# yoozzeek/zk-lisp

Hardware: AMD Instinct MI355X
Metric: segment-proofs/sec at 65536 rows, blowup=16; proof bytes bit-exact vs CPU ref (higher is better)
Workload: dtype f128 (u128 mod 2^128-45*2^40+1)

## Files before the change

### include/zkl_hip.h

```cpp
#ifndef ZKL_HIP_H
#define ZKL_HIP_H

#include <stddef.h>
#include <stdint.h>

#ifdef __cplusplus
extern "C" {
#endif

#define ZKL_ABI_VERSION 1

enum {
  ZKL_OK = 0,
  ZKL_E_INVALID = -1,
  ZKL_E_DEVICE = -2,
  ZKL_E_OOM = -3,
  ZKL_E_INTERNAL = -4,
};

typedef struct { uint64_t lo, hi; } zkl_f128;

typedef struct {
  uint32_t num_queries;
  uint32_t blowup_factor;
// ... 118 lines not shown
int zkl_hip_kernel_times(const zkl_ctx* ctx, double* out_ms, int* out_launches, int max_n, const char** names);
int zkl_hip_set_kernel_timing(zkl_ctx* ctx, int mode);

int zkl_hip_device_count(int* count);
int zkl_hip_device_alloc(zkl_ctx* ctx, size_t bytes, void** d_ptr);
int zkl_hip_device_free(zkl_ctx* ctx, void* d_ptr);
int zkl_hip_memcpy(zkl_ctx* ctx, void* dst, const void* src, size_t bytes, int kind);
int zkl_hip_synchronize(zkl_ctx* ctx);

void zkl_select_partitions(uint32_t trace_width, uint32_t trace_length,
                           uint32_t* num_partitions, uint32_t* hash_rate);

int zkl_hip_hash_rows(zkl_ctx* ctx, const void* d_matrix, uint32_t n_cols, uint32_t n_rows,
                      uint32_t num_partitions, uint32_t hash_rate, void* d_digests_out);
int zkl_hip_merkle_tree(zkl_ctx* ctx, const void* d_leaves, uint32_t n_leaves, void* d_nodes_out);
int zkl_hip_poseidon_permute(zkl_ctx* ctx, void* d_states, uint32_t n_states, int engine);
int zkl_hip_set_hash_policy(int engine, uint32_t pm_min_items);
int zkl_hip_set_row_digest_rule(int rule);
int zkl_hip_row_digest_rule(void);
int zkl_hip_set_ntt_mode(int mode);
int zkl_hip_lde(zkl_ctx* ctx, const void* d_values, uint32_t n_cols, uint32_t n_rows,
                uint32_t blowup, void* d_coeffs_out, void* d_lde_out);

#define ZKL_COL_GENERAL 0xFFFFFFFFu
int zkl_hip_set_column_structure(int on);
int zkl_hip_column_structure(void);
int zkl_hip_scan_columns(zkl_ctx* ctx, const void* d_matrix, uint32_t n_cols, uint32_t n_rows, uint32_t* period_out);
int zkl_hip_plan_row_prefix(const uint32_t* period, uint32_t n_cols, uint64_t n_lde_rows, uint32_t blowup,
                            uint32_t num_partitions, uint32_t hash_rate, uint32_t* lead_out, uint32_t* q_out,
                            uint32_t* n_parts_out);
int zkl_hip_plan_row_zero_mask(const uint32_t* period, uint32_t n_cols, uint32_t num_partitions, uint32_t hash_rate,
                               uint64_t* even_out, uint64_t* odd_out, uint32_t* n_parts_out);
int zkl_hip_set_row_zero_mask(int on);
int zkl_hip_row_zero_mask(void);
int zkl_hip_hash_rows_periodic(zkl_ctx* ctx, const void* d_matrix, uint32_t n_cols, uint32_t n_rows,
                               uint32_t num_partitions, uint32_t hash_rate, const uint32_t* row_period, int split,
                               void* d_digests_out, uint32_t* resumed_out);
int zkl_hip_lde_columns(zkl_ctx* ctx, const void* d_values, uint32_t n_cols, uint32_t n_rows, uint32_t blowup,
                        const uint32_t* period, int want_split, void* d_coeffs_out, void* d_lde_out, int* split_out);

int zkl_hip_ntt(zkl_ctx* ctx, void* d_data, uint32_t n_cols, uint32_t n, int dif, int inverse);

int zkl_verify_segment(const uint8_t* proof, size_t len, const zkl_air_public_inputs* pi,
                       const zkl_proof_options* opts);

int zkl_synth_vm_segment(uint64_t seed, uint32_t log_n, zkl_f128* trace_out,
                         zkl_air_public_inputs* pi_out, uint32_t* width_out);
#define ZKL_SYN_SPONGE 1u
#define ZKL_SYN_RAM 2u
#define ZKL_SYN_MERKLE 4u
int zkl_synth_vm_segment_ex(uint64_t seed, uint32_t log_n, uint32_t flags, zkl_f128* trace_out,
                            zkl_air_public_inputs* pi_out, uint32_t* width_out);
int zkl_synth_vm_segment_chain(uint64_t program_seed, uint64_t seed, uint32_t log_n, uint32_t flags, const zkl_f128* rom0_in,
                               zkl_f128* trace_out, zkl_air_public_inputs* pi_out, uint32_t* width_out);

enum {
  ZKL_OP_CONST = 0, ZKL_OP_MOV, ZKL_OP_ADD, ZKL_OP_SUB, ZKL_OP_MUL, ZKL_OP_NEG, ZKL_OP_EQ, ZKL_OP_SELECT,
  ZKL_OP_ASSERT, ZKL_OP_ASSERT_BIT, ZKL_OP_ASSERT_RANGE, ZKL_OP_ASSERT_RANGE_LO, ZKL_OP_ASSERT_RANGE_HI,
  ZKL_OP_DIVMOD, ZKL_OP_DIVMOD128, ZKL_OP_MULWIDE, ZKL_OP_LOAD, ZKL_OP_STORE, ZKL_OP_SABSORBN, ZKL_OP_SSQUEEZE,
  ZKL_OP_MERKLE_FIRST, ZKL_OP_MERKLE_STEP, ZKL_OP_MERKLE_LAST, ZKL_OP_END
// ... 78 lines not shown
```

### zk-lisp_amd/csrc/kernels.h

```cpp
#pragma once
#include <hip/hip_runtime.h>
#include <stdint.h>

#include <stdexcept>
#include <string>
#include "air_host.h"
#include "field.h"

namespace zkl {

struct DeviceError : std::runtime_error { using std::runtime_error::runtime_error; };
#define ZKL_HIPCHECK(x)                                                                       \
  do {                                                                                        \
    hipError_t e_ = (x);                                                                      \
    if (e_ != hipSuccess) throw ::zkl::DeviceError(std::string(#x) + ": " + hipGetErrorString(e_)); \
  } while (0)
inline void check_launch(const char* what) {
  const hipError_t e = hipGetLastError();
  if (e != hipSuccess) throw DeviceError(std::string("kernel launch failed (") + what + "): " + hipGetErrorString(e));
}

struct HasherConsts {
  fe mds[144];
  fe rc[27 * 12];
// ... 44 lines not shown
                         bool clear = true);
void decode_column_scan(const uint32_t* bits, uint32_t n_cols, size_t n_rows, uint32_t* period);
struct RowPrefixPlan {
  uint32_t np = 0;
  uint32_t lead[16] = {0};
  uint32_t q[16] = {0};
  uint64_t zeven[16] = {0};
  uint64_t zodd[16] = {0};
  bool any() const {
    for (uint32_t p = 0; p < np; p++)
      if (lead[p]) return true;
    return false;
  }
};
constexpr uint32_t ROW_MASK_PAIRS = 64;
bool row_zero_mask_enabled();
void set_row_zero_mask(bool on);
RowPrefixPlan plan_row_prefix(const uint32_t* period, uint32_t n_cols, size_t n_rows, uint32_t blowup,
                              uint32_t num_partitions, uint32_t hash_rate, size_t rows_per_entry = 64);
size_t row_prefix_table_bytes(const RowPrefixPlan& plan);
bool launch_hash_rows_prefix(const fe* d_mat, uint32_t n_cols, size_t n_rows, uint32_t num_partitions,
                             uint32_t hash_rate, const RowPrefixPlan& plan, uint32_t* d_table, fe* d_tmp, fe* d_out,
                             hipStream_t s, int split = 0);
struct OpenRowJob { uint32_t src, dst; };
struct MergeNodeJob { uint32_t left, right, dst; };
void launch_open_rows(fe* d_buf, const OpenRowJob* d_jobs, size_t njobs, uint32_t ncols, uint32_t psize, uint32_t merge,
                      hipStream_t s);
void launch_merge_jobs(fe* d_buf, const MergeNodeJob* d_jobs, size_t njobs, hipStream_t s);
void launch_merkle(fe* d_nodes, size_t n_leaves, hipStream_t s, fe* d_coin = nullptr, fe* d_root_out = nullptr,
                   int coin_mode = 0);
void launch_draws(fe seed, uint64_t base, size_t k, fe* d_out, hipStream_t s, const fe* d_seed = nullptr);
void launch_grind(fe seed, uint64_t base, uint32_t count, uint32_t bits, unsigned long long* d_best, hipStream_t s,
                  const fe* d_seed = nullptr);
void launch_fri_remainder(const fe* d_ev, uint32_t Nr, uint32_t rlen, const fe* wk, const fe* sk, fe* d_coin,
                          fe* d_rem, hipStream_t s);
void launch_query_seed(fe* d_coin, const unsigned long long* d_best, hipStream_t s);

struct MontTab {
  const uint4* l4;
  const uint32_t* l1;
};
void build_mont_table(const fe* h_w, size_t N, void* d_buf, hipStream_t s);
inline MontTab mont_tab(const void* d_buf, size_t N) {
  return MontTab{(const uint4*)d_buf, (const uint32_t*)((const char*)d_buf + N * 16)};
}
void launch_ntt_stages(fe* d_data, size_t n_cols, size_t N, bool dif, int lo_log, int hi_log,
// ... 42 lines not shown
  CeParams ce;
  fe alpha[1024];
};
struct DerivedConsts {
  fe pose_k[27];
  fe apre[1025];
  fe deep[512];
  uint32_t deep_m[512][5];
  fe deep_sz[2];
};
void launch_constraint_eval(const fe* d_lde, const fe* d_roots, size_t Ntab, const fe* d_pertab,
                            const fe* d_bm , const CeParams& p, ProofConsts* dK,
                            const DerivedConsts* dD, bool pose_block, bool ram_merkle,
                            fe* d_xinv , bool xinv_ready, fe* d_out,
                            hipStream_t s, int split = 0, fe* d_pose_part  = nullptr);
void launch_check_rows(const fe* d_trace, size_t n, const fe* d_rowper, const ProofConsts* dK, const DerivedConsts* dD,
                       bool pose_block, bool ram_merkle, fe* d_pose_part, uint32_t* d_min, hipStream_t s);
void launch_check_assertions(const fe* d_trace, size_t n, const uint32_t* d_col, const uint32_t* d_step,
                             const fe* d_val, size_t n_assert, uint32_t* d_min, hipStream_t s);
void launch_boundary_scatter(const uint32_t* d_slot, const uint32_t* d_step, const fe* d_beta, size_t n_assert,
                             size_t n, fe* d_vecs, hipStream_t s);
void launch_boundary_w(const uint32_t* d_row_start, const fe* d_beta, const fe* d_val, size_t n, fe* d_w, hipStream_t s);
void launch_check_zero_range_bitrev(const fe* d_data, size_t N, size_t lo, size_t hi, unsigned* d_flag, hipStream_t s);

struct OodArgs {
  const fe* coef;
  size_t col_stride, elem_stride, n;
  const fe* pw1;
  const fe* pw2;
  uint32_t ncols, chunks, use_off;
  uint32_t off[16];
  const uint32_t* zero;
};
void launch_ood(const OodArgs& a, fe* d_partial, hipStream_t s);
void launch_ood_frame(const fe* d_partial_trace, const fe* d_partial_comp, uint32_t W, uint32_t C, uint32_t chunks,
                      const fe* mult , fe* d_frame, hipStream_t s);
struct DeepParams {
  size_t N;
  uint32_t W, C;
  fe z, zg;
};
void launch_deep_denoms(const fe* d_roots, size_t Ntab, size_t N, fe z, fe zg, fe* d_dinv, hipStream_t s);
void launch_deep(const fe* d_lde, const fe* d_clde, const fe* d_roots, size_t Ntab, const DeepParams& p,
                 const DerivedConsts* dD, const fe* d_dinv , fe* d_out, hipStream_t s,
                 int split = 0, const uint32_t* d_list = nullptr, uint32_t n_list = 0);
void launch_fri_leaves(const fe* d_ev, size_t Nd, fe* d_leaves, hipStream_t s);
// ... 6 lines not shown
```

### zk-lisp_amd/csrc/kernels.hip

```cpp
#include <hip/hip_runtime.h>

#include <algorithm>
#include <atomic>
#include <cstdlib>
#include <cstring>
#include <map>
#include <mutex>
#include <set>
#include <stdexcept>
#include <vector>

#include "kernels.h"
#include "air_eval.h"
#include "mont26.h"

namespace zkl {


void upload_air_consts(ProofConsts* dK, const AirDevice& a, hipStream_t s) {
  ZKL_HIPCHECK(hipMemcpyAsync(&dK->air, &a, sizeof a, hipMemcpyHostToDevice, s));
}
void upload_alphas_from_device(ProofConsts* dK, const fe* d, int n, hipStream_t s) {
  if (n > 1024) throw std::invalid_argument("more than 1024 transition constraints");
  ZKL_HIPCHECK(hipMemcpyAsync(dK->alpha, d, sizeof(fe) * n, hipMemcpyDeviceToDevice, s));
// ... 1142 lines not shown
  boundary_scatter_kernel<<<(unsigned)((na + 255) / 256), 256, 0, s>>>(d_slot, d_step, d_beta, na, n, d_vecs);
}
__global__ void boundary_w_kernel(const uint32_t* rs, const fe* beta, const fe* val, size_t n, fe* w) {
  size_t row = (size_t)blockIdx.x * blockDim.x + threadIdx.x;
  if (row >= n) return;
  uint32_t acc[9] = {0, 0, 0, 0, 0, 0, 0, 0, 0};
  for (uint32_t a = rs[row]; a < rs[row + 1]; a++) mul_acc(beta[a], val[a], acc);
  w[row] = reduce288(acc);
}
void launch_boundary_w(const uint32_t* d_rs, const fe* d_beta, const fe* d_val, size_t n, fe* d_w, hipStream_t s) {
  boundary_w_kernel<<<(unsigned)((n + 255) / 256), 256, 0, s>>>(d_rs, d_beta, d_val, n, d_w);
}

__global__ void check_zero_kernel(const fe* d, size_t N, int logN, size_t lo, size_t hi, unsigned* flag) {
  size_t k = lo + (size_t)blockIdx.x * blockDim.x + threadIdx.x;
  if (k >= hi) return;
  fe v = d[bitrev((uint32_t)k, logN)];
  if (!fe_is_zero(v)) atomicOr(flag, 1u);
}
void launch_check_zero_range_bitrev(const fe* d, size_t N, size_t lo, size_t hi, unsigned* flag, hipStream_t s) {
  if (hi > lo) check_zero_kernel<<<(unsigned)((hi - lo + 255) / 256), 256, 0, s>>>(d, N, ilog2s(N), lo, hi, flag);
}

__global__ __launch_bounds__(256) void ood_kernel(OodArgs A, fe* partial) {
  const uint32_t c = blockIdx.x, k = blockIdx.z;
  if (A.zero && A.zero[c]) {
    if (threadIdx.x < 2) partial[((size_t)threadIdx.x * A.ncols + c) * A.chunks + k] = fe_zero();
    return;
  }
  const fe* col = A.coef + (A.use_off ? (size_t)A.off[c] : (size_t)c * A.col_stride);
  const size_t len = A.n / A.chunks, j0 = (size_t)k * len;
  uint32_t acc1[9] = {0, 0, 0, 0, 0, 0, 0, 0, 0}, acc2[9] = {0, 0, 0, 0, 0, 0, 0, 0, 0};
  for (size_t j = j0 + threadIdx.x; j < j0 + len; j += 256) {
    const fe v = col[j * A.elem_stride];
    mul_acc(v, A.pw1[j], acc1);
    mul_acc(v, A.pw2[j], acc2);
  }
  __shared__ fe red[2][256];
  red[0][threadIdx.x] = reduce288(acc1);
  red[1][threadIdx.x] = reduce288(acc2);
  __syncthreads();
  for (int w = 128; w > 0; w >>= 1) {
    if ((int)threadIdx.x < w) {
      red[0][threadIdx.x] = fe_add(red[0][threadIdx.x], red[0][threadIdx.x + w]);
      red[1][threadIdx.x] = fe_add(red[1][threadIdx.x], red[1][threadIdx.x + w]);
    }
// ... 187 lines not shown
```

### zk-lisp_amd/csrc/poseidon.hip

```cpp
#include <hip/hip_runtime.h>

#include <algorithm>
#include <atomic>
#include <cstdio>
#include <cstdlib>
#include <cstring>
#include <mutex>
#include <stdexcept>
#include <vector>

#include "kernels.h"
#include "mont26.h"

namespace zkl {

__constant__ HasherMont c_hm;

__device__ __forceinline__ void to_mont130(fe a, uint32_t out[5]) {
  uint32_t l[5];
  to26(a, l);
  uint64_t col[10] = {0, 0, 0, 0, 0, 0, 0, 0, 0, 0};
  mac5(l, c_hm.r2_130, col);
  redc130(col, out);
}
// ... 534 lines not shown
          if (P == COL_GENERAL || (P & (P - 1))) { ok = false; break; }
          bp = std::max<uint64_t>(bp, P);
        }
      if (!ok) break;
      lead++;
      pmax = std::max(pmax, bp);
    }
    const uint64_t q = pmax > 1 ? pmax * blowup : 1;
    if (lead && q <= nrows / rows_per_entry && (q & (q - 1)) == 0) {
      pl.lead[p] = lead;
      pl.q[p] = (uint32_t)q;
    }
  }
  return pl;
}

size_t row_prefix_table_bytes(const RowPrefixPlan& pl) {
  size_t e = 0;
  for (uint32_t p = 0; p < pl.np; p++)
    if (pl.lead[p]) e += pl.q[p];
  return e * PM_PFX_ENTRY_WORDS * sizeof(uint32_t);
}

bool launch_hash_rows_prefix(const fe* d_mat, uint32_t ncols, size_t nrows, uint32_t np, uint32_t rate,
                             const RowPrefixPlan& pl, uint32_t* d_table, fe* d_tmp, fe* d_out, hipStream_t s, int split) {
  uint32_t psize = ncols;
  if (np > 1) {
    psize = (ncols + np - 1) / np;
    if (psize < rate) psize = rate;
  }
  const uint32_t np_eff = (ncols + psize - 1) / psize;
  const bool pm_rows = hash_engine() == 1 && nrows >= pm_min_items() && np_eff <= (uint32_t)PM_PFX_PARTS && !PM_ROW_BIG_CFG;
  if (!pl.any() || !pm_rows || !d_table) {
    launch_hash_rows(d_mat, ncols, nrows, np, rate, d_tmp, d_out, s, 0, split);
    return false;
  }
  if (pl.np != np_eff) throw std::invalid_argument("launch_hash_rows_prefix: plan made for another partitioning");
  PmRowPrefix A{};
  A.table = d_table;
  uint32_t off = 0;
  size_t items = 0;
  const bool masked = row_zero_mask_enabled();
  for (uint32_t p = 0; p < np_eff; p++) {
    if (masked) {
      A.zeven[p] = pl.zeven[p];
      A.zodd[p] = pl.zodd[p];
    }
    if (!pl.lead[p]) continue;
    const uint32_t len = std::min(psize, ncols - p * psize), blocks = ((len + 1) / 2 + 1 + 9) / 10, q = pl.q[p];
    if (pl.lead[p] > blocks || q == 0 || (q & (q - 1)) || q > nrows)
      throw std::invalid_argument("launch_hash_rows_prefix: plan out of range");
    A.lead[p] = pl.lead[p];
    A.qmask[p] = q - 1;
    A.off[p] = off;
    off += q;
    items += ((size_t)q + 31) / 32 * 32;
  }
  const uint32_t merge = row_digest_rule() == 0 ? (psize != ncols) : (np_eff > 1);
  PM_GO(hash_rows_pm_table_kernel, items, false, s)(d_mat, ncols, nrows, psize, A, d_table, split);
  PM_GO(hash_rows_pm_prefix_kernel, nrows, true, s)(d_mat, ncols, nrows, psize, merge, d_out, split, A);
  return true;
}

#ifndef TOP_LDS_CFG
#define TOP_LDS_CFG 1
#endif
#ifndef TOP_WAVES_CFG
#define TOP_WAVES_CFG 4
#endif
static_assert(TOP_WAVES_CFG == 4 || TOP_WAVES_CFG == 8, "TOP_WAVES_CFG must be 4 or 8");
constexpr int TOP_WAVES = TOP_WAVES_CFG / PW_PER_WAVE;
constexpr int TOP_SLOTS = TOP_WAVES * PW_PER_WAVE;
__global__ __launch_bounds__(64 * TOP_WAVES) void merkle_top_kernel(fe* nodes, size_t lvl, int cnt, fe* coin,
                                                                    fe* root_out, int coin_mode) {
  __shared__ __align__(16) uint32_t pw_lds[TOP_WAVES * PW_WAVE_WORDS];
  __shared__ fe tn[2][TOP_SLOTS];
  PWGroup P;
  pw_init(P, pw_lds);
  const int wave_slot0 = (int)(threadIdx.x >> 6) * PW_PER_WAVE;
  const int slot = wave_slot0 + P.g;
  size_t L = lvl, base = (size_t)blockIdx.x * cnt;
  int par = 0;
// ... 202 lines not shown
```

### zk-lisp_amd/csrc/poseidon_mfma.inc

```

typedef int pm_v4i __attribute__((ext_vector_type(4)));
typedef int pm_v16i __attribute__((ext_vector_type(16)));

struct PmTables {
  int8_t afrag[6][7][64][16];
  uint64_t rk[27][12][5];
};
__device__ PmTables d_pm;

struct Pm16Tables {
  int8_t afrag[12][4][64][16];
  uint64_t rk[27][12][5];
};
__device__ Pm16Tables d_pm16;

#ifndef PM_WAVES_CFG
#define PM_WAVES_CFG 8
#endif
#ifndef PM_WIDE_CFG
#define PM_WIDE_CFG 0
#endif
constexpr int PM_WAVES = PM_WAVES_CFG;
constexpr int PM_THREADS = 64 * PM_WAVES;
#ifndef PM_ROW_WAVES_CFG
// ... 730 lines not shown
    size_t b = pm_b;
    uint32_t p = 0;
    for (; p + 1 < np; p++) {
      const size_t nb = A.lead[p] ? ((size_t)A.qmask[p] + 32) >> 5 : 0;
      if (b < nb) break;
      b -= nb;
    }
    const size_t q0 = b * 32 + (size_t)(pm_lane & 31);
    const bool live = q0 <= (size_t)A.qmask[p];
    const size_t q = live ? q0 : 0;
    const uint32_t c0 = p * psize;
    const uint32_t len = min(psize, ncols - c0);
    const fe* base = M + (size_t)c0 * nrows + lde_pos(q, nrows, split);
    uint32_t x[6][5];
    pm_sponge_init<DOM_ELEMS>(x);
    pm_sponge_blocks<false>(&tb, live, (int)((len + 1) / 2), [&](int j) {
      fe a = base[(size_t)(2 * j) * nrows];
      fe b2 = (2u * j + 1 < len) ? base[(size_t)(2 * j + 1) * nrows] : fe_zero();
      return fold_pair(a, b2);
    }, x, pm_h, 0, 10 * (int)A.lead[p]);
    if (live) {
      uint32_t* e = table + ((size_t)A.off[p] + q) * PM_PFX_ENTRY_WORDS + pm_h * 5;
#pragma unroll
      for (int T = 0; T < 6; T++)
#pragma unroll
        for (int l = 0; l < 5; l++) e[T * 10 + l] = x[T][l];
    }
  }
}

__global__ __launch_bounds__(PM_THREADS) void merkle_level_pm_kernel(fe* nodes, size_t lvl) {
  __shared__ PmTables tb;
  pm_load_tables(&tb);
  PM_LOOP(lvl) {
    const size_t it = pm_b * 32 + (size_t)(pm_lane & 31);
    const bool live = it < lvl;
    const size_t i = lvl + (live ? it : 0);
    fe d = pm_sponge<DOM_MERGE>(&tb, live, 2, [&](int j) { return nodes[2 * i + j]; });
    if (live && pm_h == 0) nodes[i] = d;
  }
}

__global__ __launch_bounds__(PM_THREADS) void fri_leaf_pm_kernel(const fe* ev, size_t half, fe* leaves) {
  __shared__ PmTables tb;
  pm_load_tables(&tb);
  PM_LOOP(half) {
    const size_t it = pm_b * 32 + (size_t)(pm_lane & 31);
    const bool live = it < half;
    const size_t i = live ? it : 0;
// ... 80 lines not shown
```

### zk-lisp_amd/csrc/prover.cpp

```cpp
#include <hip/hip_runtime.h>
#include <malloc.h>
#include <stdio.h>
#include <string.h>

#include <atomic>
#include <algorithm>
#include <chrono>
#include <functional>
#include <map>
#include <memory>
#include <mutex>
#include <set>
#include <thread>
#include <tuple>
#include <stdexcept>
#include <string>
#include <vector>

#include "../../include/zkl_hip.h"
#include "air_host.h"
#include "host_hash.h"
#include "kernels.h"
#include "lde_plan.h"
#include "host_proof.h"
// ... 65 lines not shown
    return e;
  }
  template <class T>
  T* at(size_t off = 0) const { return (T*)((char*)p + off); }
  ~HBuf() { (void)release(); }
};

}

constexpr size_t TX_CS = 48, TX_CS_MAX = 32, TX_QD = 80, TX_QD_MAX = 256, TX_FRI_SEED = 336, TX_WORDS = 344;

struct zkl_ctx {
  int device = 0;
  hipStream_t stream = nullptr;
  std::mutex mu;
  std::string err;
  double stage_ms[ZKL_NUM_STAGES] = {0};
  double host_ms[3] = {0, 0, 0};
  size_t tab_n = 0, tab_N = 0;
  DBuf roots, iroots, mroots, miroots, opow, opow_n, pertab;
  DBuf trace, coef, lde, parts, tree, ce, bvec, bm, clde, ctree, deep, draws, pw, oodv, oodf, txs, asl, ast, asv, ars;
  DBuf lcoef;
  DBuf fri_ev, fri_tree, best, gaddr, gout, flag;
  DBuf xinv;
  DBuf posep;
  DBuf cexinv;
  size_t cexinv_key_n = 0, cexinv_key_ce = 0, cexinv_key_tab = 0;
  const void* cexinv_key_roots = nullptr;
  DBuf scanbits, pfxtab, colmeta, psmall;
  HBuf h_scan, h_meta;
  ZeroBook zero_known, zero_stage;
  DBuf kconst;
  DBuf dconst;
  DBuf fri_coin;
  HBuf h_asrt, h_ood, h_addr, h_gv, h_tx, h_air;
  hipStream_t aux = nullptr;
  hipEvent_t aux_ev = nullptr, hev = nullptr;
  hipStream_t up = nullptr;
  std::vector<void*> up_slot;
  std::vector<hipEvent_t> up_ev;
  size_t up_slot_bytes = 0;
  double up_ms = 0;
  hipEvent_t stage_ev[ZKL_NUM_STAGES + 1] = {};
  bool stage_ev_ready = false;
  size_t pert_key_n = 0, pert_key_ce = 0;
  std::vector<hipEvent_t> evpool;
  std::vector<std::pair<int, size_t>> kmarks;
  size_t evnext = 0;
  int ktiming = 1;
  double kfam_ms[ZKL_NUM_KFAMILIES] = {0};
  int kfam_n[ZKL_NUM_KFAMILIES] = {0};
  std::vector<uint8_t> proof_s;
// ... 92 lines not shown
    C->iroots.ensure(N * sizeof(fe));
    HIPCHECK(hipMemcpyAsync(C->roots.p, w.data(), N * sizeof(fe), hipMemcpyHostToDevice, s));
    HIPCHECK(hipMemcpyAsync(C->iroots.p, wi.data(), N * sizeof(fe), hipMemcpyHostToDevice, s));
    C->mroots.ensure(N * 20);
    C->miroots.ensure(N * 20);
    build_mont_table(w.data(), N, C->mroots.p, s);
    build_mont_table(wi.data(), N, C->miroots.p, s);
    HIPCHECK(hipStreamSynchronize(s));
    C->tab_N = N;
  }
  if (C->tab_n != n) {
    std::vector<fe> o(n), on(n);
    fe inv_n = fe_inv(fe{n, 0}), p = fe_one();
    for (size_t k = 0; k < n; k++) { o[k] = p; on[k] = fe_mul(p, inv_n); p = fe_mul(p, fe{3, 0}); }
    C->opow.ensure(n * sizeof(fe));
    C->opow_n.ensure(n * sizeof(fe));
    HIPCHECK(hipMemcpyAsync(C->opow.p, o.data(), n * sizeof(fe), hipMemcpyHostToDevice, s));
    HIPCHECK(hipMemcpyAsync(C->opow_n.p, on.data(), n * sizeof(fe), hipMemcpyHostToDevice, s));
    HIPCHECK(hipStreamSynchronize(s));
    C->tab_n = n;
  }
}

struct StageTimer {
  zkl_ctx* C;
  hipEvent_t* ev;
  bool inner;
  explicit StageTimer(zkl_ctx* c) : C(c), ev(c->stage_ev), inner(c->ktiming == 2) {
    if (!C->stage_ev_ready) {
      for (int i = 0; i <= ZKL_NUM_STAGES; i++) HIPCHECK(hipEventCreate(&C->stage_ev[i]));
      C->stage_ev_ready = true;
    }
  }
  void mark(int i) {
    if (inner || i == 0 || i == ZKL_NUM_STAGES) HIPCHECK(hipEventRecord(ev[i], C->stream));
  }
  void finish() {
    HIPCHECK(hipEventSynchronize(ev[ZKL_NUM_STAGES]));
    for (int i = 0; i < ZKL_NUM_STAGES; i++) {
      float ms = 0;
      if (inner) HIPCHECK(hipEventElapsedTime(&ms, ev[i], ev[i + 1]));
      C->stage_ms[i] = ms;
    }
  }
};

// ... 273 lines not shown
      KScope k(C, KF_MISC);
      launch_scan_columns((const fe*)d_trace_in, W, n, (uint32_t*)C->scanbits.p, s);
      check_launch("column scan");
      read_scan();
    }
    KScope k(C, KF_NTT);
    split = trace_lde_columns(C, book, (const fe*)d_trace_in, W, n, N, colstruct ? period.data() : nullptr, C->coef.f(),
                              C->lde.f(), g_lde_split, &meta, s);
  }
  check_launch("trace LDE");
  if (split < 0) split = 0;
  T.mark(1);
  C->parts.ensure((size_t)o.num_partitions * N * sizeof(fe) + N * sizeof(fe));
  C->tree.ensure(2 * N * sizeof(fe));
  if (colstruct && trace_on_host) {
    read_scan();
    ZeroBook none;
    meta = upload_col_meta(C, plan_structured_lde(period.data(), W, n, none), W, B, s);
  }
  {
    RowPrefixPlan plan;
    if (colstruct) plan = plan_row_prefix(period.data(), W, N, B, o.num_partitions, o.hash_rate);
    if (plan.any()) C->pfxtab.ensure(row_prefix_table_bytes(plan));
    KScope k(C, KF_TRACE_HASH);
    launch_hash_rows_prefix(C->lde.f(), W, N, o.num_partitions, o.hash_rate, plan, (uint32_t*)C->pfxtab.p, C->parts.f(),
                            C->tree.f() + N, s, split);
  }
  check_launch("trace row hash");
  std::vector<fe> seed_el = context_elements(W, n, o);
  auto pie = pi_elements(pi);
  seed_el.insert(seed_el.end(), pie.begin(), pie.end());
  Coin coin{H.hash_elements(seed_el.data(), seed_el.size()), 0};
  C->txs.ensure(64 * sizeof(fe));
  C->h_tx.ensure(TX_WORDS * sizeof(fe));
  fe* tx = C->txs.f();
  fe* htx = C->h_tx.at<fe>();
  htx[32] = coin.seed;
  HIPCHECK(hipMemcpyAsync(tx, htx + 32, sizeof(fe), hipMemcpyHostToDevice, s));
  {
    KScope k(C, KF_MERKLE);
    launch_merkle(C->tree.f(), N, s, tx, tx + 2, 1);
  }
  check_launch("trace Merkle tree and trace-root reseed");
  coin.counter = 0;
  AirInstance& air = C->air;
  {
// ... 100 lines not shown
      p = fe_mul(p, wb);
    }
  }
  cp.n_bcols = nb;
  for (uint32_t u = 0; u < nb; u++) cp.bcol[u] = bcols[u];
  C->ce.ensure(ce * sizeof(fe));
  {
    KScope k(C, KF_CEVAL);
    const bool ready = C->cexinv_key_n == n && C->cexinv_key_ce == ce && C->cexinv_key_tab == Ntab &&
                       C->cexinv_key_roots == (const void*)roots && C->cexinv.bytes >= ce * sizeof(fe);
    if (!ready) {
      C->cexinv_key_n = 0;
      C->cexinv.ensure(ce * sizeof(fe));
    }
    if (air.dev.pose_block) C->posep.ensure(ce * sizeof(fe));
    launch_constraint_eval(C->lde.f(), roots, Ntab, C->pertab.f(), C->bm.f(), cp, dK, dD, air.dev.pose_block != 0,
                           (air.dev.ram_block | air.dev.merkle_block) != 0, C->cexinv.f(), ready, C->ce.f(), s, split,
                           air.dev.pose_block ? C->posep.f() : nullptr);
    C->cexinv_key_n = n; C->cexinv_key_ce = ce; C->cexinv_key_tab = Ntab; C->cexinv_key_roots = roots;
  }
  check_launch("constraint evaluation");
  T.mark(3);

  C->flag.ensure(16);
  C->clde.ensure((size_t)Cc * N * sizeof(fe));
  const int loge = ilog2(ce / n);
  const fe inv3 = fe_inv(three), inv_ce = fe_inv(fe{ce, 0});
  {
    KScope k(C, KF_NTT);
    launch_ntt_stages(C->ce.f(), 1, ce, true, 0, logce - 1, miroots, Ntab, s);
    HIPCHECK(hipMemsetAsync(C->flag.p, 0, 4, s));
    launch_check_zero_range_bitrev(C->ce.f(), ce, (size_t)Cc * n, ce, (unsigned*)C->flag.p, s);
    for (int j = 0; j < Cc; j++) {
      fe mult = fe_mul(fe_pow64(inv3, (uint64_t)j * n), inv_ce);
      launch_broadcast(C->ce.f(), 0, ce / n, bitrev_u((uint32_t)j, loge), 1, n, n, nullptr, mult, false,
                       C->lcoef.f() + (size_t)j * n, s);
    }
    launch_lde_from_coeffs(C->lcoef.f(), Cc, n, N, mroots, Ntab, C->clde.f(), s, false);
  }
  check_launch("composition polynomial LDE");
  C->ctree.ensure(2 * N * sizeof(fe));
  {
    KScope k(C, KF_COMP_HASH);
    launch_hash_rows(C->clde.f(), Cc, N, o.num_partitions, o.hash_rate, C->parts.f(), C->ctree.f() + N, s, 1);
  }
  {
    KScope k(C, KF_MERKLE);
    launch_merkle(C->ctree.f(), N, s, tx, tx + 3, 1);
  }
  check_launch("composition commitment");
  HIPCHECK(hipMemcpyAsync(htx, tx, 4 * sizeof(fe), hipMemcpyDeviceToHost, s));
  HIPCHECK(hipMemcpyAsync(htx + 4, C->flag.p, 4, hipMemcpyDeviceToHost, s));
  HIPCHECK(hipStreamSynchronize(s));
  HT("croot");
  unsigned bad = 0;
  memcpy(&bad, htx + 4, 4);
  if (bad) throw InvalidArg("constraint composition polynomial degree too large: trace does not satisfy the AIR");
  const fe troot = htx[2], croot = htx[3];
  coin.seed = htx[0];
  coin.counter = 0;
  T.mark(4);

  fe z = coin.draw(), zg = fe_mul(z, g);
  C->pw.ensure(4 * n * sizeof(fe));
  fe* pw = C->pw.f();
  powers_kernel<<<(unsigned)((n + 255) / 256), 256, 0, s>>>(fe_mul(z, inv3), fe_one(), n, logn, pw + 2 * n);
  powers_kernel<<<(unsigned)((n + 255) / 256), 256, 0, s>>>(fe_mul(zg, inv3), fe_one(), n, logn, pw + 3 * n);
  const uint32_t chunks = n >= 8192 ? 32 : 1;
  const size_t n_otr = 2 * (size_t)W * chunks, n_ocp = 2 * (size_t)Cc * chunks;
  C->oodv.ensure((n_otr + n_ocp) * sizeof(fe));
  fe* dood = C->oodv.f();
  if (Cc > 16) throw std::runtime_error("internal: more than 16 composition columns");
  {
    KScope k(C, KF_MISC);
    OodArgs a{};
    a.coef = C->coef.f(); a.col_stride = n; a.elem_stride = 1; a.n = n;
    a.pw1 = pw + 2 * n; a.pw2 = pw + 3 * n; a.ncols = W; a.chunks = chunks; a.use_off = 0;
    a.zero = meta.zero;
    launch_ood(a, dood, s);
    OodArgs b{};
    b.coef = C->ce.f(); b.col_stride = 0; b.elem_stride = ce / n; b.n = n;
    b.pw1 = pw + 2 * n; b.pw2 = pw + 3 * n; b.ncols = (uint32_t)Cc; b.chunks = chunks; b.use_off = 1;
    for (int j = 0; j < Cc; j++) b.off[j] = bitrev_u((uint32_t)j, loge);
    launch_ood(b, dood + n_otr, s);
  }
  std::vector<fe> cmult(Cc);
  for (int j = 0; j < Cc; j++) cmult[j] = fe_mul(fe_pow64(inv3, (uint64_t)j * n), inv_ce);
  C->oodf.ensure(2 * ((size_t)W + Cc) * sizeof(fe));
  fe* dframe = C->oodf.f();
  launch_ood_frame(dood, dood + n_otr, W, (uint32_t)Cc, chunks, cmult.data(), dframe, s);
  check_launch("OOD evaluation");
  const size_t nfr = 2 * ((size_t)W + Cc);
  C->h_ood.ensure(nfr * sizeof(fe));
  const fe* frame = C->h_ood.at<fe>();
  HIPCHECK(hipMemcpyAsync(C->h_ood.p, dframe, nfr * sizeof(fe), hipMemcpyDeviceToHost, s));
// ... 1035 lines not shown
}

int zkl_hip_row_zero_mask(void) { return row_zero_mask_enabled() ? 1 : 0; }

int zkl_hip_hash_rows_periodic(zkl_ctx* c, const void* d_m, uint32_t nc, uint32_t nr, uint32_t np, uint32_t rate,
                               const uint32_t* row_period, int split, void* d_out, uint32_t* resumed_out) {
  if (resumed_out) *resumed_out = 0;
  if (!c || !d_m || !d_out || !row_period || nc == 0 || np < 1 || np > 16 || rate < 1 || rate > 256 || split < 0 ||
      split > 1 || (split && (nr < 2048 || (nr & (nr - 1)))))
    return ZKL_E_INVALID;
  std::lock_guard<std::mutex> lk(c->mu);
  return run_guarded(c, [&] {
    c->zero_stage.forget();
    HIPCHECK(hipSetDevice(c->device));
    upload_hasher(c->stream);
    c->parts.ensure((size_t)std::max<uint32_t>(np, 1) * nr * sizeof(fe) + 16);
    RowPrefixPlan plan;
    if (column_structure_enabled()) plan = plan_row_prefix(row_period, nc, nr, 1, np, rate, 1);
    if (plan.any()) c->pfxtab.ensure(row_prefix_table_bytes(plan));
    const bool used = launch_hash_rows_prefix((const fe*)d_m, nc, nr, np, rate, plan, (uint32_t*)c->pfxtab.p,
                                              c->parts.f(), (fe*)d_out, c->stream, split);
    if (used && resumed_out)
      for (uint32_t p = 0; p < plan.np; p++) *resumed_out += plan.lead[p] != 0;
    check_launch("stage entry point");
    HIPCHECK(hipStreamSynchronize(c->stream));
  });
}

int zkl_hip_lde_columns(zkl_ctx* c, const void* d_values, uint32_t nc, uint32_t n, uint32_t blowup,
                        const uint32_t* period, int want_split, void* d_coeffs, void* d_lde, int* split_out) {
  if (!c || !d_values || !d_coeffs || !d_lde || nc == 0 || nc > 4096 || n < 2 || (n & (n - 1)) || blowup < 2 ||
      (blowup & (blowup - 1)))
    return ZKL_E_INVALID;
  std::lock_guard<std::mutex> lk(c->mu);
  return run_guarded(c, [&] {
    HIPCHECK(hipSetDevice(c->device));
    const size_t N = (size_t)n * blowup;
    ensure_tables(c, n, N);
    hipStream_t s = c->stream;
    std::vector<uint32_t> per(nc, COL_GENERAL);
    if (column_structure_enabled()) {
      if (period) {
        per.assign(period, period + nc);
      } else {
        c->scanbits.ensure((size_t)nc * sizeof(uint32_t));
        c->h_scan.ensure((size_t)nc * sizeof(uint32_t));
        launch_scan_columns((const fe*)d_values, nc, n, (uint32_t*)c->scanbits.p, s);
// ... 95 lines not shown
    HIPCHECK(hipMemcpyAsync(coef, d_values, (size_t)nc * n * sizeof(fe), hipMemcpyDeviceToDevice, s));
    launch_ntt_stages(coef, nc, n, true, 0, ilog2(n) - 1, mont_tab(c->miroots.p, c->tab_N), c->tab_N, s);
    launch_scale_bitrev(coef, nc, n, c->opow_n.f(), s);
    launch_lde_from_coeffs(coef, nc, n, N, mont_tab(c->mroots.p, c->tab_N), c->tab_N, (fe*)d_lde, s);
    check_launch("stage entry point");
    std::vector<fe> h((size_t)nc * n), r((size_t)nc * n);
    HIPCHECK(hipMemcpyAsync(h.data(), coef, h.size() * sizeof(fe), hipMemcpyDeviceToHost, s));
    HIPCHECK(hipStreamSynchronize(s));
    const fe inv3 = fe_inv(fe{3, 0});
    int logn = ilog2(n);
    std::vector<fe> i3k(n);
    i3k[0] = fe_one();
    for (uint32_t k = 1; k < n; k++) i3k[k] = fe_mul(i3k[k - 1], inv3);
    for (uint32_t col = 0; col < nc; col++)
      for (uint32_t j = 0; j < n; j++) {
        const uint32_t k = bitrev_u(j, logn);
        r[(size_t)col * n + k] = fe_mul(h[(size_t)col * n + j], i3k[k]);
      }
    HIPCHECK(hipMemcpyAsync(coef, r.data(), r.size() * sizeof(fe), hipMemcpyHostToDevice, s));
    HIPCHECK(hipStreamSynchronize(s));
  });
}

}
```

### zk-lisp_amd/zkl_hip/__init__.py

```python
from __future__ import annotations

import ctypes as C
import os

__all__ = [
    "F128", "ProofOptions", "AirPublicInputs", "ZklError", "Context", "load_library",
    "select_partitions_for_trace", "proof_options", "synth_vm_segment", "STAGE_NAMES",
    "FM_VM", "FM_VM_EXPECT", "FM_POSEIDON", "FM_SPONGE", "FM_MERKLE", "FM_RAM",
    "VmArg", "StepInfo", "check_request", "row_digest_rule", "verify_segment", "step_proof_encode", "step_proof_digest", "parse_step_proof", "children_root",
    "AggOptions", "agg_prove", "agg_verify", "agg_trace", "parse_agg_artifact", "synth_segment_chain", "synth_vm_segment_chain",
    "step_info_for", "ZklOp", "op", "build_trace", "OP_KINDS", "rom_acc_from_program", "plan_segments", "slice_segment",
]

_HERE = os.path.dirname(os.path.abspath(__file__))
LIB_PATH = os.path.join(_HERE, "libzkl_hip.so")

FM_POSEIDON, FM_VM, FM_VM_EXPECT, FM_SPONGE, FM_MERKLE, FM_RAM = 1, 2, 16, 32, 64, 128

STAGE_NAMES = ["trace_lde", "trace_commit", "evaluator", "constraint_commitment", "ood",
               "deep", "fri", "grind", "queries", "finish"]

ERRORS = {-1: "invalid", -2: "device", -3: "oom", -4: "internal"}


# ... 142 lines not shown
    lib.zkl_hip_device_alloc.argtypes = [C.c_void_p, C.c_size_t, P(C.c_void_p)]
    lib.zkl_hip_device_free.argtypes = [C.c_void_p, C.c_void_p]
    lib.zkl_hip_memcpy.argtypes = [C.c_void_p, C.c_void_p, C.c_void_p, C.c_size_t, C.c_int]
    lib.zkl_hip_synchronize.argtypes = [C.c_void_p]
    lib.zkl_select_partitions.argtypes = [C.c_uint32, C.c_uint32, P(C.c_uint32), P(C.c_uint32)]
    lib.zkl_synth_vm_segment.argtypes = [C.c_uint64, C.c_uint32, C.c_void_p, P(AirPublicInputs), P(C.c_uint32)]
    lib.zkl_synth_vm_segment_ex.argtypes = [C.c_uint64, C.c_uint32, C.c_uint32, C.c_void_p, P(AirPublicInputs),
                                            P(C.c_uint32)]
    lib.zkl_hip_ntt.argtypes = [C.c_void_p, C.c_void_p, C.c_uint32, C.c_uint32, C.c_int, C.c_int]
    lib.zkl_hip_hash_rows.argtypes = [C.c_void_p, C.c_void_p, C.c_uint32, C.c_uint32, C.c_uint32, C.c_uint32, C.c_void_p]
    lib.zkl_hip_merkle_tree.argtypes = [C.c_void_p, C.c_void_p, C.c_uint32, C.c_void_p]
    lib.zkl_hip_poseidon_permute.argtypes = [C.c_void_p, C.c_void_p, C.c_uint32, C.c_int]
    lib.zkl_hip_set_hash_policy.argtypes = [C.c_int, C.c_uint32]
    lib.zkl_hip_set_ntt_mode.argtypes = [C.c_int]
    lib.zkl_hip_set_row_digest_rule.argtypes = [C.c_int]
    lib.zkl_verify_segment.argtypes = [C.c_char_p, C.c_size_t, P(AirPublicInputs), P(ProofOptions)]
    lib.zkl_hip_check_request.argtypes = [C.c_uint32, C.c_uint32, P(AirPublicInputs), P(ProofOptions)]
    lib.zkl_hip_set_kernel_timing.argtypes = [C.c_void_p, C.c_int]
    lib.zkl_step_proof_encode.argtypes = [P(AirPublicInputs), P(StepInfo), C.c_char_p, C.c_size_t,
                                          P(P(C.c_uint8)), P(C.c_size_t)]
    lib.zkl_step_proof_digest.argtypes = [C.c_char_p, C.c_size_t, C.c_void_p, C.c_void_p]
    lib.zkl_children_root.argtypes = [C.c_char_p, C.c_char_p, C.c_char_p, C.c_uint32, C.c_void_p]
    lib.zkl_hip_lde.argtypes = [C.c_void_p, C.c_void_p, C.c_uint32, C.c_uint32, C.c_uint32, C.c_void_p, C.c_void_p]
    lib.zkl_hip_set_column_structure.argtypes = [C.c_int]
    lib.zkl_hip_column_structure.argtypes = []
    lib.zkl_hip_scan_columns.argtypes = [C.c_void_p, C.c_void_p, C.c_uint32, C.c_uint32, P(C.c_uint32)]
    lib.zkl_hip_plan_row_prefix.argtypes = [P(C.c_uint32), C.c_uint32, C.c_uint64, C.c_uint32, C.c_uint32, C.c_uint32,
                                            P(C.c_uint32), P(C.c_uint32), P(C.c_uint32)]
    lib.zkl_hip_plan_row_zero_mask.argtypes = [P(C.c_uint32), C.c_uint32, C.c_uint32, C.c_uint32, P(C.c_uint64),
                                               P(C.c_uint64), P(C.c_uint32)]
    lib.zkl_hip_set_row_zero_mask.argtypes = [C.c_int]
    lib.zkl_hip_row_zero_mask.argtypes = []
    lib.zkl_hip_hash_rows_periodic.argtypes = [C.c_void_p, C.c_void_p, C.c_uint32, C.c_uint32, C.c_uint32, C.c_uint32,
                                               P(C.c_uint32), C.c_int, C.c_void_p, P(C.c_uint32)]
    lib.zkl_hip_lde_columns.argtypes = [C.c_void_p, C.c_void_p, C.c_uint32, C.c_uint32, C.c_uint32, P(C.c_uint32),
                                        C.c_int, C.c_void_p, C.c_void_p, P(C.c_int)]
    lib.zkl_synth_vm_segment_chain.argtypes = [C.c_uint64, C.c_uint64, C.c_uint32, C.c_uint32, P(F128), C.c_void_p,
                                               P(AirPublicInputs), P(C.c_uint32)]
    lib.zkl_build_trace.argtypes = [C.c_void_p, C.c_uint32, C.c_char_p, C.c_char_p, C.c_void_p, C.c_uint32, C.c_void_p,
                                    C.c_uint32, P(F128), C.c_void_p, P(AirPublicInputs), P(C.c_uint32),
                                    P(C.c_uint32)]
    lib.zkl_rom_acc_from_program.argtypes = [C.c_void_p, C.c_uint32, C.c_char_p, P(F128)]
    lib.zkl_plan_segments.argtypes = [C.c_uint32, C.c_uint32, P(C.c_uint32), P(C.c_uint32), C.c_uint32, P(C.c_uint32)]
    lib.zkl_slice_segment.argtypes = [C.c_void_p, C.c_uint32, C.c_uint32, C.c_void_p, C.c_uint32, P(AirPublicInputs),
                                      C.c_uint32, C.c_uint32, C.c_void_p, P(AirPublicInputs), P(C.c_uint32),
                                      C.c_void_p, C.c_void_p]
# ... 900 lines not shown
```

Baseline: 22.92.

## Fuse composition zero-check and scatter; add lane-per-row prefix table kernel

Replaces the per-column broadcast launches and the separate zero-range check with one comp_scatter kernel. It scales the composition coefficients and flags nonzero high-degree terms in a single pass. A flag mark counter replaces the per-proof memset. A wave-per-item Poseidon prefix-table kernel is added and used by default when the table is small, with table entries canonicalized so both paths produce the same bytes. Test and debug entry points are also added; the main cost is extra code paths that must stay bit-exact.

```diff
diff --git a/include/zkl_hip.h b/include/zkl_hip.h
--- a/include/zkl_hip.h
+++ b/include/zkl_hip.h
@@ -164,6 +164,9 @@
 int zkl_hip_lde(zkl_ctx* ctx, const void* d_values, uint32_t n_cols, uint32_t n_rows,
                 uint32_t blowup, void* d_coeffs_out, void* d_lde_out);
 
+int zkl_hip_comp_scatter(zkl_ctx* ctx, const void* d_ce, uint32_t n, uint32_t ce, uint32_t n_cols, int fused,
+                         void* d_coeffs_out, uint32_t* failed_out);
+
 #define ZKL_COL_GENERAL 0xFFFFFFFFu
 int zkl_hip_set_column_structure(int on);
 int zkl_hip_column_structure(void);
@@ -178,6 +181,9 @@
 int zkl_hip_hash_rows_periodic(zkl_ctx* ctx, const void* d_matrix, uint32_t n_cols, uint32_t n_rows,
                                uint32_t num_partitions, uint32_t hash_rate, const uint32_t* row_period, int split,
                                void* d_digests_out, uint32_t* resumed_out);
+int zkl_hip_set_row_table_form(int form);
+int zkl_hip_row_table_form(void);
+int zkl_hip_last_row_prefix_table(zkl_ctx* ctx, void* buf, size_t cap, size_t* len);
 int zkl_hip_lde_columns(zkl_ctx* ctx, const void* d_values, uint32_t n_cols, uint32_t n_rows, uint32_t blowup,
                         const uint32_t* period, int want_split, void* d_coeffs_out, void* d_lde_out, int* split_out);
 
diff --git a/zk-lisp_amd/csrc/kernels.h b/zk-lisp_amd/csrc/kernels.h
--- a/zk-lisp_amd/csrc/kernels.h
+++ b/zk-lisp_amd/csrc/kernels.h
@@ -90,6 +90,9 @@
 bool launch_hash_rows_prefix(const fe* d_mat, uint32_t n_cols, size_t n_rows, uint32_t num_partitions,
                              uint32_t hash_rate, const RowPrefixPlan& plan, uint32_t* d_table, fe* d_tmp, fe* d_out,
                              hipStream_t s, int split = 0);
+constexpr size_t ROW_TABLE_LANE_MAX = 2048;
+int row_table_form();
+void set_row_table_form(int form);
 struct OpenRowJob { uint32_t src, dst; };
 struct MergeNodeJob { uint32_t left, right, dst; };
 void launch_open_rows(fe* d_buf, const OpenRowJob* d_jobs, size_t njobs, uint32_t ncols, uint32_t psize, uint32_t merge,
@@ -178,6 +181,11 @@
                              size_t n, fe* d_vecs, hipStream_t s);
 void launch_boundary_w(const uint32_t* d_row_start, const fe* d_beta, const fe* d_val, size_t n, fe* d_w, hipStream_t s);
 void launch_check_zero_range_bitrev(const fe* d_data, size_t N, size_t lo, size_t hi, unsigned* d_flag, hipStream_t s);
+struct CompScatter {
+  fe mult[16];
+};
+void launch_comp_scatter(const fe* d_ce, size_t n, size_t ce, uint32_t C, const CompScatter& A, fe* d_out,
+                         unsigned* d_flag, unsigned mark, hipStream_t s);
 
 struct OodArgs {
   const fe* coef;
diff --git a/zk-lisp_amd/csrc/kernels.hip b/zk-lisp_amd/csrc/kernels.hip
--- a/zk-lisp_amd/csrc/kernels.hip
+++ b/zk-lisp_amd/csrc/kernels.hip
@@ -1188,6 +1188,28 @@
   if (hi > lo) check_zero_kernel<<<(unsigned)((hi - lo + 255) / 256), 256, 0, s>>>(d, N, ilog2s(N), lo, hi, flag);
 }
 
+__global__ void comp_scatter_kernel(const fe* __restrict__ d, int logn, int loge, uint32_t C, CompScatter A,
+                                    fe* __restrict__ out, unsigned* flag, unsigned mark) {
+  const size_t i = (size_t)blockIdx.x * blockDim.x + threadIdx.x;
+  if (i >= ((size_t)1 << (logn + loge))) return;
+  const uint32_t j = (uint32_t)(i >> logn);
+  const size_t k = i & (((size_t)1 << logn) - 1);
+  fe v = d[bitrev(j, loge) + (k << loge)];
+  if (j < C) {
+    const fe mult = A.mult[j];
+    if (!(mult.lo == 1 && mult.hi == 0)) v = fe_mul(v, mult);
+    out[i] = v;
+  } else if (!fe_is_zero(v)) {
+    atomicExch(flag, mark);
+  }
+}
+void launch_comp_scatter(const fe* d_ce, size_t n, size_t ce, uint32_t C, const CompScatter& A, fe* d_out,
+                         unsigned* d_flag, unsigned mark, hipStream_t s) {
+  if (C > 16 || ce < n || (size_t)C * n > ce) throw std::invalid_argument("launch_comp_scatter: bad column count");
+  comp_scatter_kernel<<<(unsigned)((ce + 255) / 256), 256, 0, s>>>(d_ce, ilog2s(n), ilog2s(ce / n), C, A, d_out, d_flag,
+                                                                  mark);
+}
+
 __global__ __launch_bounds__(256) void ood_kernel(OodArgs A, fe* partial) {
   const uint32_t c = blockIdx.x, k = blockIdx.z;
   if (A.zero && A.zero[c]) {
diff --git a/zk-lisp_amd/csrc/poseidon.hip b/zk-lisp_amd/csrc/poseidon.hip
--- a/zk-lisp_amd/csrc/poseidon.hip
+++ b/zk-lisp_amd/csrc/poseidon.hip
@@ -580,6 +580,61 @@
   return e * PM_PFX_ENTRY_WORDS * sizeof(uint32_t);
 }
 
+__global__ __launch_bounds__(256) void hash_rows_pw_table_kernel(const fe* __restrict__ M, uint32_t ncols, size_t nrows,
+                                                                 uint32_t psize, PmRowPrefix A,
+                                                                 uint32_t* __restrict__ table, int split) {
+  PW_SETUP();
+  const uint32_t np = (ncols + psize - 1) / psize;
+  size_t q = item;
+  uint32_t p = 0, maxlead = 0;
+  bool found = false;
+  for (uint32_t k = 0; k < np; k++) {
+    maxlead = max(maxlead, A.lead[k]);
+    const size_t nq = A.lead[k] ? (size_t)A.qmask[k] + 1 : 0;
+    if (!found && q < nq) {
+      found = true;
+      p = k;
+    }
+    if (!found) q -= nq;
+  }
+  const bool live = P.g < PW_PER_WAVE && found;
+  if (!live) p = 0, q = 0;
+  const uint32_t c0 = p * psize;
+  const uint32_t len = min(psize, ncols - c0), lead = A.lead[p];
+  const int total = (int)((len + 1) / 2) + 1;
+  const fe* base = M + (size_t)c0 * nrows + lde_pos(q, nrows, split);
+  uint32_t s[5];
+#pragma unroll
+  for (int l = 0; l < 5; l++)
+    s[l] = P.e == 0 ? c_hm.dfe130[DOM_ELEMS][l] : P.e == 10 ? c_hm.dom130[0][l] : P.e == 11 ? c_hm.dom130[1][l] : 0u;
+  for (uint32_t b = 0; b < maxlead; b++) {
+    const int idx = (int)b * 10 + P.e;
+    if (live && b < lead && P.e < 10 && idx >= 1 && idx < total) {
+      const uint32_t j = (uint32_t)idx - 1;
+      const fe a = base[(size_t)(2 * j) * nrows];
+      const fe b2 = (2 * j + 1 < len) ? base[(size_t)(2 * j + 1) * nrows] : fe_zero();
+      uint32_t m[5];
+      to_mont130(fold_pair(a, b2), m);
+#pragma unroll
+      for (int l = 0; l < 5; l++) s[l] += m[l];
+    }
+    pw_permute(P, s);
+    if (b + 1 == lead) {
+      uint32_t c[5];
+      to_mont130(from_mont130(s), c);
+      if (live && P.h == 0) {
+        uint32_t* e = table + ((size_t)A.off[p] + q) * PM_PFX_ENTRY_WORDS + P.e * 5;
+#pragma unroll
+        for (int l = 0; l < 5; l++) e[l] = c[l];
+      }
+    }
+  }
+}
+
+static std::atomic<int> g_row_table_form{0};
+int row_table_form() { return g_row_table_form.load(); }
+void set_row_table_form(int form) { g_row_table_form.store(form); }
+
 bool launch_hash_rows_prefix(const fe* d_mat, uint32_t ncols, size_t nrows, uint32_t np, uint32_t rate,
                              const RowPrefixPlan& pl, uint32_t* d_table, fe* d_tmp, fe* d_out, hipStream_t s, int split) {
   uint32_t psize = ncols;
@@ -615,7 +670,11 @@
     items += ((size_t)q + 31) / 32 * 32;
   }
   const uint32_t merge = row_digest_rule() == 0 ? (psize != ncols) : (np_eff > 1);
-  PM_GO(hash_rows_pm_table_kernel, items, false, s)(d_mat, ncols, nrows, psize, A, d_table, split);
+  const int form = row_table_form();
+  if (form == 2 || (form == 0 && off <= ROW_TABLE_LANE_MAX))
+    hash_rows_pw_table_kernel<<<pw_blocks(off), 256, 0, s>>>(d_mat, ncols, nrows, psize, A, d_table, split);
+  else
+    PM_GO(hash_rows_pm_table_kernel, items, false, s)(d_mat, ncols, nrows, psize, A, d_table, split);
   PM_GO(hash_rows_pm_prefix_kernel, nrows, true, s)(d_mat, ncols, nrows, psize, merge, d_out, split, A);
   return true;
 }
diff --git a/zk-lisp_amd/csrc/poseidon_mfma.inc b/zk-lisp_amd/csrc/poseidon_mfma.inc
--- a/zk-lisp_amd/csrc/poseidon_mfma.inc
+++ b/zk-lisp_amd/csrc/poseidon_mfma.inc
@@ -776,9 +776,12 @@
     if (live) {
       uint32_t* e = table + ((size_t)A.off[p] + q) * PM_PFX_ENTRY_WORDS + pm_h * 5;
 #pragma unroll
-      for (int T = 0; T < 6; T++)
-#pragma unroll
-        for (int l = 0; l < 5; l++) e[T * 10 + l] = x[T][l];
+      for (int T = 0; T < 6; T++) {
+        uint32_t c[5];
+        to_mont130(from_mont130(x[T]), c);
+#pragma unroll
+        for (int l = 0; l < 5; l++) e[T * 10 + l] = c[l];
+      }
     }
   }
 }
diff --git a/zk-lisp_amd/csrc/prover.cpp b/zk-lisp_amd/csrc/prover.cpp
--- a/zk-lisp_amd/csrc/prover.cpp
+++ b/zk-lisp_amd/csrc/prover.cpp
@@ -111,12 +111,14 @@
   DBuf trace, coef, lde, parts, tree, ce, bvec, bm, clde, ctree, deep, draws, pw, oodv, oodf, txs, asl, ast, asv, ars;
   DBuf lcoef;
   DBuf fri_ev, fri_tree, best, gaddr, gout, flag;
+  uint32_t flag_mark = 0;
   DBuf xinv;
   DBuf posep;
   DBuf cexinv;
   size_t cexinv_key_n = 0, cexinv_key_ce = 0, cexinv_key_tab = 0;
   const void* cexinv_key_roots = nullptr;
   DBuf scanbits, pfxtab, colmeta, psmall;
+  size_t pfxtab_used = 0;
   HBuf h_scan, h_meta;
   ZeroBook zero_known, zero_stage;
   DBuf kconst;
@@ -255,6 +257,15 @@
   }
 }
 
+unsigned next_flag_mark(zkl_ctx* C, hipStream_t s) {
+  if (!C->flag.p || C->flag_mark == UINT32_MAX) {
+    C->flag.ensure(16);
+    HIPCHECK(hipMemsetAsync(C->flag.p, 0, 16, s));
+    C->flag_mark = 0;
+  }
+  return ++C->flag_mark;
+}
+
 struct StageTimer {
   zkl_ctx* C;
   hipEvent_t* ev;
@@ -574,6 +585,7 @@
     RowPrefixPlan plan;
     if (colstruct) plan = plan_row_prefix(period.data(), W, N, B, o.num_partitions, o.hash_rate);
     if (plan.any()) C->pfxtab.ensure(row_prefix_table_bytes(plan));
+    C->pfxtab_used = 0;
     KScope k(C, KF_TRACE_HASH);
     launch_hash_rows_prefix(C->lde.f(), W, N, o.num_partitions, o.hash_rate, plan, (uint32_t*)C->pfxtab.p, C->parts.f(),
                             C->tree.f() + N, s, split);
@@ -720,20 +732,17 @@
   check_launch("constraint evaluation");
   T.mark(3);
 
-  C->flag.ensure(16);
+  const unsigned flag_mark = next_flag_mark(C, s);
+  if (Cc > 16) throw std::runtime_error("internal: more than 16 composition columns");
   C->clde.ensure((size_t)Cc * N * sizeof(fe));
   const int loge = ilog2(ce / n);
   const fe inv3 = fe_inv(three), inv_ce = fe_inv(fe{ce, 0});
   {
     KScope k(C, KF_NTT);
     launch_ntt_stages(C->ce.f(), 1, ce, true, 0, logce - 1, miroots, Ntab, s);
-    HIPCHECK(hipMemsetAsync(C->flag.p, 0, 4, s));
-    launch_check_zero_range_bitrev(C->ce.f(), ce, (size_t)Cc * n, ce, (unsigned*)C->flag.p, s);
-    for (int j = 0; j < Cc; j++) {
-      fe mult = fe_mul(fe_pow64(inv3, (uint64_t)j * n), inv_ce);
-      launch_broadcast(C->ce.f(), 0, ce / n, bitrev_u((uint32_t)j, loge), 1, n, n, nullptr, mult, false,
-                       C->lcoef.f() + (size_t)j * n, s);
-    }
+    CompScatter cs{};
+    for (int j = 0; j < Cc; j++) cs.mult[j] = fe_mul(fe_pow64(inv3, (uint64_t)j * n), inv_ce);
+    launch_comp_scatter(C->ce.f(), n, ce, (uint32_t)Cc, cs, C->lcoef.f(), (unsigned*)C->flag.p, flag_mark, s);
     launch_lde_from_coeffs(C->lcoef.f(), Cc, n, N, mroots, Ntab, C->clde.f(), s, false);
   }
   check_launch("composition polynomial LDE");
@@ -753,7 +762,7 @@
   HT("croot");
   unsigned bad = 0;
   memcpy(&bad, htx + 4, 4);
-  if (bad) throw InvalidArg("constraint composition polynomial degree too large: trace does not satisfy the AIR");
+  if (bad == flag_mark) throw InvalidArg("constraint composition polynomial degree too large: trace does not satisfy the AIR");
   const fe troot = htx[2], croot = htx[3];
   coin.seed = htx[0];
   coin.counter = 0;
@@ -768,7 +777,6 @@
   const size_t n_otr = 2 * (size_t)W * chunks, n_ocp = 2 * (size_t)Cc * chunks;
   C->oodv.ensure((n_otr + n_ocp) * sizeof(fe));
   fe* dood = C->oodv.f();
-  if (Cc > 16) throw std::runtime_error("internal: more than 16 composition columns");
   {
     KScope k(C, KF_MISC);
     OodArgs a{};
@@ -1850,7 +1858,28 @@
                                               c->parts.f(), (fe*)d_out, c->stream, split);
     if (used && resumed_out)
       for (uint32_t p = 0; p < plan.np; p++) *resumed_out += plan.lead[p] != 0;
+    c->pfxtab_used = used ? row_prefix_table_bytes(plan) : 0;
     check_launch("stage entry point");
+    HIPCHECK(hipStreamSynchronize(c->stream));
+  });
+}
+
+int zkl_hip_set_row_table_form(int form) {
+  if (form < 0 || form > 2) return ZKL_E_INVALID;
+  set_row_table_form(form);
+  return 0;
+}
+
+int zkl_hip_row_table_form(void) { return row_table_form(); }
+
+int zkl_hip_last_row_prefix_table(zkl_ctx* c, void* buf, size_t cap, size_t* len) {
+  if (!c || !len || (!buf && cap)) return ZKL_E_INVALID;
+  std::lock_guard<std::mutex> lk(c->mu);
+  return run_guarded(c, [&] {
+    *len = c->pfxtab_used;
+    if (!c->pfxtab_used || cap < c->pfxtab_used) return;
+    HIPCHECK(hipSetDevice(c->device));
+    HIPCHECK(hipMemcpyAsync(buf, c->pfxtab.p, c->pfxtab_used, hipMemcpyDeviceToHost, c->stream));
     HIPCHECK(hipStreamSynchronize(c->stream));
   });
 }
@@ -1992,4 +2021,37 @@
   });
 }
 
-}
+int zkl_hip_comp_scatter(zkl_ctx* c, const void* d_ce, uint32_t n, uint32_t ce, uint32_t n_cols, int fused,
+                         void* d_coeffs_out, uint32_t* failed_out) {
+  if (!c || !d_ce || !d_coeffs_out || !failed_out || n < 1 || (n & (n - 1)) || ce < n || (ce & (ce - 1)) || n_cols < 1 ||
+      n_cols > 16 || (uint64_t)n_cols * n > ce || fused < 0 || fused > 1)
+    return ZKL_E_INVALID;
+  std::lock_guard<std::mutex> lk(c->mu);
+  return run_guarded(c, [&] {
+    c->zero_stage.forget();
+    HIPCHECK(hipSetDevice(c->device));
+    hipStream_t s = c->stream;
+    const int loge = ilog2(ce / n);
+    const fe inv3 = fe_inv(fe{3, 0}), inv_ce = fe_inv(fe{ce, 0});
+    CompScatter cs{};
+    for (uint32_t j = 0; j < n_cols; j++) cs.mult[j] = fe_mul(fe_pow64(inv3, (uint64_t)j * n), inv_ce);
+    unsigned mark = next_flag_mark(c, s), got = 0;
+    if (fused) {
+      launch_comp_scatter((const fe*)d_ce, n, ce, n_cols, cs, (fe*)d_coeffs_out, (unsigned*)c->flag.p, mark, s);
+    } else {
+      mark = 1;
+      HIPCHECK(hipMemsetAsync(c->flag.p, 0, 4, s));
+      launch_check_zero_range_bitrev((const fe*)d_ce, ce, (size_t)n_cols * n, ce, (unsigned*)c->flag.p, s);
+      for (uint32_t j = 0; j < n_cols; j++)
+        launch_broadcast((const fe*)d_ce, 0, ce / n, bitrev_u(j, loge), 1, n, n, nullptr, cs.mult[j], false,
+                         (fe*)d_coeffs_out + (size_t)j * n, s);
+    }
+    check_launch("stage entry point");
+    HIPCHECK(hipMemcpyAsync(&got, c->flag.p, 4, hipMemcpyDeviceToHost, s));
+    if (!fused) HIPCHECK(hipMemsetAsync(c->flag.p, 0, 4, s));
+    HIPCHECK(hipStreamSynchronize(s));
+    *failed_out = got == mark;
+  });
+}
+
+}
diff --git a/zk-lisp_amd/zkl_hip/__init__.py b/zk-lisp_amd/zkl_hip/__init__.py
--- a/zk-lisp_amd/zkl_hip/__init__.py
+++ b/zk-lisp_amd/zkl_hip/__init__.py
@@ -188,6 +188,12 @@
     lib.zkl_step_proof_digest.argtypes = [C.c_char_p, C.c_size_t, C.c_void_p, C.c_void_p]
     lib.zkl_children_root.argtypes = [C.c_char_p, C.c_char_p, C.c_char_p, C.c_uint32, C.c_void_p]
     lib.zkl_hip_lde.argtypes = [C.c_void_p, C.c_void_p, C.c_uint32, C.c_uint32, C.c_uint32, C.c_void_p, C.c_void_p]
+    if hasattr(lib, "zkl_hip_comp_scatter"):
+        lib.zkl_hip_comp_scatter.argtypes = [C.c_void_p, C.c_void_p, C.c_uint32, C.c_uint32, C.c_uint32, C.c_int,
+                                             C.c_void_p, P(C.c_uint32)]
+        lib.zkl_hip_set_row_table_form.argtypes = [C.c_int]
+        lib.zkl_hip_row_table_form.argtypes = []
+        lib.zkl_hip_last_row_prefix_table.argtypes = [C.c_void_p, C.c_void_p, C.c_size_t, P(C.c_size_t)]
     lib.zkl_hip_set_column_structure.argtypes = [C.c_int]
     lib.zkl_hip_column_structure.argtypes = []
     lib.zkl_hip_scan_columns.argtypes = [C.c_void_p, C.c_void_p, C.c_uint32, C.c_uint32, P(C.c_uint32)]
```

Result: no change. 22.90 (median of 2 runs) (-0.1%).
